# simonfuhrmann/mve

Measured on NVIDIA H100. Metric: mvs_depth_pixels_per_second, higher is better.
Workload: dtype f32

## Files before the change

mve_b200/csrc/b200mvs.cu:

```cuda
#include "../../include/b200mvs.h"
#include "patch_opt.cuh"
#include "patch_warp.cuh"
#include "patch_thread.cuh"

#include <algorithm>
#include <cmath>
#include <cstdarg>
#include <cstdio>
#include <cstring>
#include <cstdlib>
#include <map>
#include <chrono>
#include <ctime>
#include <mutex>
#include <string>
#include <thread>
#include <atomic>
#include <vector>

using namespace b200mvs;

namespace {

thread_local std::string g_create_error;
// ... 941 lines not shown
    {
        same_camera = v.valid && !v.lv.empty() && v.w == w && v.h == h && v.flen == flen && v.paspect == paspect && v.pp[0] == pp[0] && v.pp[1] == pp[1] &&
                      std::memcmp(v.rot, rot, sizeof(v.rot)) == 0 && std::memcmp(v.trans, trans, sizeof(v.trans)) == 0;
        if (!same_camera) { std::lock_guard<std::mutex> pl(ctx->plan_mtx); ctx->plans.clear(); }
    }
    if (!same_camera) {
        v.valid = false;
        v.has_image = false;
        v.w = w; v.h = h; v.flen = flen; v.paspect = paspect; v.pp[0] = pp[0]; v.pp[1] = pp[1];
        std::memcpy(v.rot, rot, sizeof(v.rot));
        std::memcpy(v.trans, trans, sizeof(v.trans));
        v.campos[0] = -rot[0] * trans[0] - rot[3] * trans[1] - rot[6] * trans[2];
        v.campos[1] = -rot[1] * trans[0] - rot[4] * trans[1] - rot[7] * trans[2];
        v.campos[2] = -rot[2] * trans[0] - rot[5] * trans[1] - rot[8] * trans[2];
        for (int r = 0; r < 3; ++r) {
            v.w2c[4 * r] = rot[3 * r]; v.w2c[4 * r + 1] = rot[3 * r + 1]; v.w2c[4 * r + 2] = rot[3 * r + 2]; v.w2c[4 * r + 3] = trans[r];
        }
        v.lv.clear();
        float ppx = pp[0], ppy = pp[1];
        int cw = w, chh = h;
        auto push_level = [&]() {
            HostLevel L; L.w = cw; L.h = chh; L.pitch = (cw + 3) & ~3;
            fill_calibration(v, ppx, ppy, (float)cw, (float)chh, L.proj, L.invproj);
            v.lv.push_back(L);
        };
        push_level();
        while (std::min(cw, chh) >= 30) {
            if (cw % 2 == 1) ppx = ppx * float(cw) / float(cw + 1);
            if (chh % 2 == 1) ppy = ppy * float(chh) / float(chh + 1);
            cw = (cw + 1) / 2; chh = (chh + 1) / 2;
            push_level();
        }
    }
    if ((int)v.lv.size() > MAX_LEVELS) return fail(ctx, B200MVS_ERR_UNSUPPORTED, "image too large: %d pyramid levels", (int)v.lv.size());
    if (!d_src) {
        if (v.d_base) { cudaFree(v.d_base); v.d_base = nullptr; v.bytes = 0; }
        v.has_image = false;
        v.valid = true;
        ctx->views_dirty = true;
        return 0;
    }
    size_t total = 0;
    for (HostLevel& L : v.lv) total += (size_t)L.pitch * L.h;
    const size_t need = total * (sizeof(uchar4) + sizeof(uint4));
    if (!v.d_base || v.bytes != need) {
        if (v.d_base) { cudaFree(v.d_base); v.d_base = nullptr; }
        CK(cudaMalloc(&v.d_base, need));
        v.bytes = need;
        ctx->views_dirty = true;
    }
    size_t off = 0;
    uint4* qbase = reinterpret_cast<uint4*>(v.d_base + total);
    for (HostLevel& L : v.lv) { L.d_img = v.d_base + off; L.d_quad = qbase + off; off += (size_t)L.pitch * L.h; }
    const dim3 blk(32, 8);
    k_import_rgb<<<dim3((w + 31) / 32, (h + 7) / 8), blk, 0, stream>>>(d_src, w, h, ch, v.lv[0].d_img, v.lv[0].pitch);
    const float w1 = std::exp(-0.5f / (2.0f * 1.0f)), w2 = std::exp(-2.5f / (2.0f * 1.0f)), w3 = std::exp(-4.5f / (2.0f * 1.0f));
    for (size_t i = 1; i < v.lv.size(); ++i) {
        const HostLevel& a = v.lv[i - 1];
        const HostLevel& b = v.lv[i];
        k_half_gaussian<<<dim3((b.w + 31) / 32, (b.h + 7) / 8), blk, 0, stream>>>(a.d_img, a.w, a.h, a.pitch, b.d_img, b.w, b.h, b.pitch, w1, w2, w3);
    }
    for (const HostLevel& L : v.lv)
        k_make_quads<<<dim3((L.w + 31) / 32, (L.h + 7) / 8), blk, 0, stream>>>(L.d_img, L.w, L.h, L.pitch, L.d_quad);
    CK(cudaGetLastError());
    v.valid = true;
    v.has_image = true;
    ctx->views_dirty = true;
    return 0;
}

int sync_view_params(b200mvs_ctx* ctx)
{
    if (!ctx->views_dirty) return 0;
    std::vector<ViewParams> hp(ctx->views.size());
    std::memset(hp.data(), 0, hp.size() * sizeof(ViewParams));
    for (size_t i = 0; i < ctx->views.size(); ++i) {
        const HostView& v = ctx->views[i];
        ViewParams& p = hp[i];
        p.valid = v.valid ? 1 : 0;
        if (!v.valid) continue;
        std::memcpy(p.campos, v.campos, 12);
        std::memcpy(p.w2c, v.w2c, 48);
        std::memcpy(p.rot, v.rot, 36);
        p.inv_ax0 = v.lv[0].invproj[0];
        p.nlevels = (int)v.lv.size();
        for (size_t l = 0; l < v.lv.size(); ++l) {
            const HostLevel& L = v.lv[l];
            p.lv[l].ax = L.proj[0]; p.lv[l].ay = L.proj[4]; p.lv[l].cx = L.proj[2]; p.lv[l].cy = L.proj[5];
            p.lv[l].w = L.w; p.lv[l].h = L.h; p.lv[l].pitch = L.pitch; p.lv[l].img = v.has_image ? L.d_img : nullptr;
            p.lv[l].quad = v.has_image ? L.d_quad : nullptr;
        }
    }
    CK(cudaMemcpyAsync(ctx->d_views, hp.data(), hp.size() * sizeof(ViewParams), cudaMemcpyHostToDevice, ctx->stream));
    CK(cudaStreamSynchronize(ctx->stream));
    ctx->views_dirty = false;
    return 0;
}

cudaEvent_t get_event(b200mvs_ctx* ctx, size_t i)
{
    while (ctx->ev_pool.size() <= i) { cudaEvent_t e; cudaEventCreate(&e); ctx->ev_pool.push_back(e); }
    return ctx->ev_pool[i];
}

int prepare_kernels(b200mvs_ctx* ctx)
{
    if (ctx->frontier_grid) return 0;
    CK(cudaFuncSetAttribute(k_frontier, cudaFuncAttributeMaxDynamicSharedMemorySize, (int)OPT_SMEM_BYTES));
    CK(cudaFuncSetAttribute(k_optimize, cudaFuncAttributeMaxDynamicSharedMemorySize, (int)OPT_SMEM_BYTES));
    int per_sm = 0, per_sm_opt = 0, sms = 0;
    CK(cudaOccupancyMaxActiveBlocksPerMultiprocessor(&per_sm, k_frontier, OPT_TPB, OPT_SMEM_BYTES));
    CK(cudaOccupancyMaxActiveBlocksPerMultiprocessor(&per_sm_opt, k_optimize, OPT_TPB, OPT_SMEM_BYTES));
    CK(cudaDeviceGetAttribute(&sms, cudaDevAttrMultiProcessorCount, ctx->device));
    if (per_sm < 1 || per_sm_opt < 1) return fail(ctx, B200MVS_ERR_CUDA, "patch-optimisation kernels do not fit on an SM");
    ctx->optimize_grid = per_sm_opt * sms;
    ctx->frontier_grid = per_sm * sms;
    return 0;
}

int make_job(b200mvs_ctx* ctx, const b200mvs_settings& s, int ref, const std::vector<int>& gsel, JobParams& J)
{
    const HostView& rv = ctx->views[ref];
    if (s.scale >= (int)rv.lv.size()) return fail(ctx, B200MVS_ERR_INVALID_ARG, "Invalid scale factor");
    const HostLevel& L = rv.lv[s.scale];
    std::memset(&J, 0, sizeof(J));
    J.ref_view = ref; J.W = L.w; J.H = L.h; J.n_global = (int)gsel.size();
    for (size_t k = 0; k < gsel.size(); ++k) J.gview[k] = gsel[k];
    J.ki0 = L.invproj[0]; J.ki2 = L.invproj[2]; J.ki4 = L.invproj[4]; J.ki5 = L.invproj[5];
    J.ref_img = L.d_img; J.ref_pitch = L.pitch;
    return 0;
}

unsigned ids_to_slots(const std::vector<int>& gsel, const int32_t* ids, int n, bool* ok)
{
    unsigned s = 0xFFFFFFFFu;
    std::vector<int> slots;
    for (int k = 0; k < n; ++k) {
        auto it = std::lower_bound(gsel.begin(), gsel.end(), (int)ids[k]);
        if (it == gsel.end() || *it != ids[k]) { *ok = false; return s; }
        slots.push_back((int)(it - gsel.begin()));
    }
    std::sort(slots.begin(), slots.end());
    for (size_t k = 0; k < slots.size() && k < 4; ++k) s = (s & ~(0xFFu << (8 * k))) | ((unsigned)slots[k] << (8 * k));
    *ok = true;
    return s;
}

}

extern "C" {

const char* b200mvs_version(void) { return "b200mvs 0.1 (sm_90a)"; }

void b200mvs_default_settings(b200mvs_settings* s)
{
    if (!s) return;
    s->filter_width = 5; s->min_ncc = 0.3f; s->min_parallax = 10.0f; s->accept_ncc = 0.6f; s->min_refine_diff = 0.001f;
    s->max_iterations = 20; s->nr_recon_neighbors = 4; s->global_vs_max = 20; s->scale = 0; s->use_color_scale = 1;
    for (int i = 0; i < 3; ++i) { s->aabb_min[i] = -3.402823466e+38f; s->aabb_max[i] = 3.402823466e+38f; }
    s->frontier_band = 0.f; s->frontier_topk = 0;
}

const char* b200mvs_last_error(const b200mvs_ctx* ctx) { return ctx ? ctx->err.c_str() : g_create_error.c_str(); }

int b200mvs_create(int device, int n_views, b200mvs_ctx** out)
{
    b200mvs_ctx* ctx = nullptr;
    if (!out || n_views <= 0) return fail(nullptr, B200MVS_ERR_INVALID_ARG, "b200mvs_create: bad arguments");
    *out = nullptr;
    if (device == B200MVS_DEVICE_NONE) {
        ctx = new b200mvs_ctx();
        ctx->device = B200MVS_DEVICE_NONE;
        ctx->views.resize(n_views);
        *out = ctx;
        return 0;
    }
    int ndev = 0;
    cudaError_t e = cudaGetDeviceCount(&ndev);
    if (e != cudaSuccess || ndev == 0)
        return fail(nullptr, B200MVS_ERR_CUDA, "no CUDA device available (%s); b200mvs has no CPU fallback", cudaGetErrorString(e));
    if (device < 0 || device >= ndev) return fail(nullptr, B200MVS_ERR_INVALID_ARG, "device %d out of range (%d devices)", device, ndev);
    e = cudaSetDevice(device);
    if (e != cudaSuccess) return fail(nullptr, B200MVS_ERR_CUDA, "cudaSetDevice: %s", cudaGetErrorString(e));
    ctx = new b200mvs_ctx();
    ctx->device = device;
    ctx->views.resize(n_views);
    auto bail = [&](const char* what, cudaError_t ce) {
        fail(nullptr, B200MVS_ERR_CUDA, "%s: %s", what, cudaGetErrorString(ce));
        delete ctx;
        return B200MVS_ERR_CUDA;
    };
    if ((e = cudaStreamCreateWithFlags(&ctx->stream, cudaStreamNonBlocking)) != cudaSuccess) return bail("cudaStreamCreate", e);
    if ((e = cudaMalloc(&ctx->d_views, sizeof(ViewParams) * n_views)) != cudaSuccess) return bail("cudaMalloc(views)", e);
    if ((e = cudaMalloc(&ctx->d_lut, 256 * sizeof(float))) != cudaSuccess) return bail("cudaMalloc(lut)", e);
    if ((e = cudaMallocHost(&ctx->h_counters, sizeof(unsigned long long) * 4096)) != cudaSuccess) return bail("cudaMallocHost", e);
    if ((e = cudaHostAlloc(&ctx->h_mirror, sizeof(unsigned long long) * 8192, cudaHostAllocMapped)) != cudaSuccess) return bail("cudaHostAlloc", e);
    float lut[256];
    for (int i = 0; i < 256; ++i) {
        const double x = i / 255.0;
        lut[i] = (float)((i <= 0.04045 * 255.0) ? x / 12.92 : std::pow((x + 0.055) / 1.055, 2.4));
    }
    if ((e = cudaMemcpy(ctx->d_lut, lut, sizeof(lut), cudaMemcpyHostToDevice)) != cudaSuccess) return bail("cudaMemcpy(lut)", e);
    *out = ctx;
    return 0;
}

void b200mvs_destroy(b200mvs_ctx* ctx)
{
    if (!ctx) return;
    if (ctx->device == B200MVS_DEVICE_NONE) { delete ctx; return; }
    cudaSetDevice(ctx->device);
    for (HostView& v : ctx->views) if (v.d_base) cudaFree(v.d_base);
    if (ctx->d_views) cudaFree(ctx->d_views);
    if (ctx->d_lut) cudaFree(ctx->d_lut);
    if (ctx->h_counters) cudaFreeHost(ctx->h_counters);
    if (ctx->h_mirror) cudaFreeHost(ctx->h_mirror);
    for (b200mvs_ctx::Stage& S : ctx->stage) {
        if (S.host) cudaFreeHost(S.host);
        if (S.dev) cudaFree(S.dev);
        if (S.done) cudaEventDestroy(S.done);
    }
    ctx->ent_a.release(); ctx->ent_b.release(); ctx->run_in.release(); ctx->run_sorted.release(); ctx->tile_cnt.release(); ctx->tile_off.release(); ctx->run_out.release(); ctx->written.release();
    ctx->counters.release(); ctx->d_jobs.release(); ctx->d_settings.release(); ctx->maps.release();
    ctx->ctl.release(); ctx->hist.release(); ctx->thr_bin.release(); ctx->job_cancel.release(); ctx->job_run.release();
    for (cudaEvent_t e : ctx->ev_pool) cudaEventDestroy(e);
    if (ctx->stream) cudaStreamDestroy(ctx->stream);
    delete ctx;
}

int b200mvs_upload_view(b200mvs_ctx* ctx, int id, const uint8_t* rgb, int w, int h, int channels,
                        float flen, float paspect, const float ppoint[2], const float rot[9], const float trans[3])
{
    if (!ctx) return B200MVS_ERR_INVALID_ARG;
    std::lock_guard<std::mutex> lk(ctx->mtx);
    if (ctx->device == B200MVS_DEVICE_NONE) return fail(ctx, B200MVS_ERR_CUDA, "planning context (B200MVS_DEVICE_NONE): no CUDA device, b200mvs has no CPU fallback");
    if (id < 0 || id >= (int)ctx->views.size() || !rgb || w < 2 || h < 2 || !ppoint || !rot || !trans)
        return fail(ctx, B200MVS_ERR_INVALID_ARG, "b200mvs_upload_view: bad arguments");
    if (channels < 1 || channels > 4) return fail(ctx, B200MVS_ERR_INVALID_ARG, "Image with invalid number of channels");
    CK(cudaSetDevice(ctx->device));
    const size_t bytes = (size_t)w * h * channels;
    b200mvs_ctx::Stage& S = ctx->stage[ctx->stage_next++ & 1u];
    if (S.busy) { CK(cudaEventSynchronize(S.done)); S.busy = false; }
    if (S.cap < bytes) {
        if (S.host) cudaFreeHost(S.host);
        if (S.dev) cudaFree(S.dev);
        S.host = nullptr; S.dev = nullptr; S.cap = 0;
        CK(cudaMallocHost(&S.host, bytes));
        CK(cudaMalloc(&S.dev, bytes));
        S.cap = bytes;
    }
    if (!S.done) CK(cudaEventCreateWithFlags(&S.done, cudaEventDisableTiming));
    std::memcpy(S.host, rgb, bytes);
    CK(cudaMemcpyAsync(S.dev, S.host, bytes, cudaMemcpyHostToDevice, ctx->stream));
    const int rc = upload_common(ctx, id, S.dev, w, h, channels, flen, paspect, ppoint, rot, trans, ctx->stream);
    CK(cudaEventRecord(S.done, ctx->stream));
    S.busy = true;
    return rc;
}

int b200mvs_upload_view_device(b200mvs_ctx* ctx, int id, const uint8_t* rgb_dev, int w, int h,
                               float flen, float paspect, const float ppoint[2], const float rot[9], const float trans[3],
                               void* cuda_stream)
{
    if (!ctx) return B200MVS_ERR_INVALID_ARG;
    std::lock_guard<std::mutex> lk(ctx->mtx);
    if (ctx->device == B200MVS_DEVICE_NONE) return fail(ctx, B200MVS_ERR_CUDA, "planning context (B200MVS_DEVICE_NONE): no CUDA device, b200mvs has no CPU fallback");
    if (id < 0 || id >= (int)ctx->views.size() || !rgb_dev || w < 2 || h < 2 || !ppoint || !rot || !trans)
        return fail(ctx, B200MVS_ERR_INVALID_ARG, "b200mvs_upload_view_device: bad arguments");
    CK(cudaSetDevice(ctx->device));
    cudaStream_t s = cuda_stream ? (cudaStream_t)cuda_stream : ctx->stream;
    int rc = upload_common(ctx, id, rgb_dev, w, h, 3, flen, paspect, ppoint, rot, trans, s);
    cudaError_t e = cudaStreamSynchronize(s);
    if (!rc && e != cudaSuccess) rc = fail(ctx, B200MVS_ERR_CUDA, "upload sync: %s", cudaGetErrorString(e));
    return rc;
}

int b200mvs_set_view_camera(b200mvs_ctx* ctx, int id, int w, int h, float flen, float paspect, const float ppoint[2],
                            const float rot[9], const float trans[3])
{
    if (!ctx) return B200MVS_ERR_INVALID_ARG;
    std::lock_guard<std::mutex> lk(ctx->mtx);
    if (id < 0 || id >= (int)ctx->views.size() || w < 2 || h < 2 || !ppoint || !rot || !trans)
        return fail(ctx, B200MVS_ERR_INVALID_ARG, "b200mvs_set_view_camera: bad arguments");
    if (ctx->device != B200MVS_DEVICE_NONE) CK(cudaSetDevice(ctx->device));
    return upload_common(ctx, id, nullptr, w, h, 3, flen, paspect, ppoint, rot, trans, ctx->stream);
}

int b200mvs_set_features(b200mvs_ctx* ctx, int n, const float* pos, const int32_t* off, const int32_t* ids)
{
    if (!ctx) return B200MVS_ERR_INVALID_ARG;
    std::lock_guard<std::mutex> lk(ctx->mtx);
    if (n < 0 || (n > 0 && (!pos || !off || !ids))) return fail(ctx, B200MVS_ERR_INVALID_ARG, "b200mvs_set_features: bad arguments");
    { std::lock_guard<std::mutex> pl(ctx->plan_mtx); ctx->plans.clear(); }
    ctx->feats.resize(n);
    for (int i = 0; i < n; ++i) {
        std::memcpy(ctx->feats[i].pos, pos + 3 * i, 12);
        ctx->feats[i].refs.assign(ids + off[i], ids + off[i + 1]);
    }
    ctx->view_feats.assign(ctx->views.size(), std::vector<int>());
    for (int i = 0; i < n; ++i)
        for (int vid : ctx->feats[i].refs)
            if (vid >= 0 && vid < (int)ctx->views.size()) {
                std::vector<int>& vf = ctx->view_feats[vid];
                if (vf.empty() || vf.back() != i) vf.push_back(i);
            }
    return 0;
// ... 452 lines not shown
```

mve_b200/csrc/patch_thread.cuh:

```cuda
#pragma once
#include "patch_opt.cuh"

namespace b200mvs {

struct PatchT {
    const DevSettings* st;
    const ViewParams* views;
#if defined(B200MVS_HOST_EMU)
    const float* lut_tab;
    unsigned lane4;
#endif
    const JobParams* job;
    unsigned xy;
    float u0x, u0y, u0z;
    float uax, uay, uaz;
    float ubx, uby, ubz;
    float c0x, c0y, c0z;
    float mx0, mx1, mx2;
    float crx, cry, crz;
    float cpx, cpy, cpz;
    float mfp, inv_mfp;
    float mm, inv_mm, sqrDevX;
    float depth, dzI, dzJ;
    unsigned avail;
    int iter;
    unsigned n_sets;
    unsigned pk;
    unsigned selp;
    float cs[MAX_LOCAL][3];
    float ncc[MAX_LOCAL];


    struct PassOut { float num, den, nX0, nX1, nX2; };
    enum Stage { LVS_CTOR, CTOR, FIRST, PRE, POST, LVS_REPL, REPL, DONE };
    enum : unsigned {
        F_REF_OK = 1u << 0,
        F_OPTI = 1u << 1, F_CONVERGED = 1u << 2, F_LVS_OK = 1u << 3, F_VIEW_REMOVED = 1u << 4, F_WAS_NORMAL = 1u << 5,
        F_NORMAL = 1u << 6, F_SINGULAR = 1u << 7, F_HAS_NORMAL = 1u << 8, F_HAS_NCC = 1u << 9
    };
    static constexpr int SH_STAGE = 10, SH_NSEL = 13, SH_COL = 16, SH_DER = 20, SH_DF = 24;
    __device__ __forceinline__ bool is(unsigned f) const { return (pk & f) != 0u; }
    __device__ __forceinline__ void put(unsigned f, bool v) { pk = v ? (pk | f) : (pk & ~f); }
    __device__ __forceinline__ int stage() const { return (int)((pk >> SH_STAGE) & 7u); }
    __device__ __forceinline__ void set_stage(int v) { pk = (pk & ~(7u << SH_STAGE)) | ((unsigned)v << SH_STAGE); }
    __device__ __forceinline__ int nsel() const { return (int)((pk >> SH_NSEL) & 7u); }
    __device__ __forceinline__ void set_nsel(int v) { pk = (pk & ~(7u << SH_NSEL)) | ((unsigned)v << SH_NSEL); }
    __device__ __forceinline__ int sel(int k) const { return (int)((selp >> (8 * k)) & 0xFFu); }
    __device__ __forceinline__ int px() const { return (int)(xy & 0xFFFFu); }
    __device__ __forceinline__ int py() const { return (int)(xy >> 16); }

    template <typename T> static __device__ __forceinline__ T get4(const T (&a)[MAX_LOCAL], int k)
    {
        return k == 0 ? a[0] : (k == 1 ? a[1] : (k == 2 ? a[2] : a[3]));
    }
    template <typename T> static __device__ __forceinline__ void set4(T (&a)[MAX_LOCAL], int k, T v)
    {
#pragma unroll
        for (int i = 0; i < MAX_LOCAL; ++i) if (i == k) a[i] = v;
    }

    __device__ __forceinline__ unsigned lane_offset() const
    {
#if defined(B200MVS_HOST_EMU)
        return lane4;
#else
        return (threadIdx.x & 31u) << 2;
#endif
    }
    __device__ __forceinline__ const float* table() const
    {
#if defined(B200MVS_HOST_EMU)
        return lut_tab;
#else
        extern __shared__ float b200mvs_dyn_smem[];
        return b200mvs_dyn_smem;
#endif
    }

    __device__ __forceinline__ void sample_ray(float di, float dj, float& ux, float& uy, float& uz, float& inv) const
    {
        ux = u0x + di * uax + dj * ubx;
        uy = u0y + di * uay + dj * uby;
        uz = u0z + di * uaz + dj * ubz;
        inv = rsqrt_fast(ux * ux + uy * uy + uz * uz);
    }

    __device__ __forceinline__ void compute_points()
    {
        bool bad = false;
#pragma unroll 5
        for (int k = 0; k < NS; ++k) {
            const float t = depth + (float)(k % 5 - 2) * dzI + (float)(k / 5 - 2) * dzJ;
            bad |= t <= 0.f;
        }
        if (bad) pk &= ~F_REF_OK;
        cpx = c0x + depth * crx;
        cpy = c0y + depth * cry;
        cpz = c0z + depth * crz;
        const ViewParams* rv = &views[job->ref_view];
        const float z = __ldg(&rv->w2c[8]) * cpx + __ldg(&rv->w2c[9]) * cpy + __ldg(&rv->w2c[10]) * cpz + __ldg(&rv->w2c[11]);
        mfp = z * job->ki0;
        inv_mfp = rcp_fast(mfp);
    }

    __device__ __forceinline__ void init_sampler(int x, int y)
    {
        const float* const lut_tab = table();
        const unsigned lane4 = lane_offset();
        pk &= ~F_REF_OK; mm = 0.f; inv_mm = 0.f; sqrDevX = 0.f;
        mx0 = mx1 = mx2 = 0.f;
        crx = cry = crz = cpx = cpy = cpz = mfp = inv_mfp = 0.f;
        if (x - 2 < 0 || y - 2 < 0 || x + 2 > job->W - 1 || y + 2 > job->H - 1) return;
        {
            const ViewParams* rv = &views[job->ref_view];
            const float r0 = __ldg(&rv->rot[0]), r1 = __ldg(&rv->rot[1]), r2 = __ldg(&rv->rot[2]), r3 = __ldg(&rv->rot[3]), r4 = __ldg(&rv->rot[4]);
            const float r5 = __ldg(&rv->rot[5]), r6 = __ldg(&rv->rot[6]), r7 = __ldg(&rv->rot[7]), r8 = __ldg(&rv->rot[8]);
            const float vx = job->ki0 * ((float)x + 0.5f) + job->ki2, vy = job->ki4 * ((float)y + 0.5f) + job->ki5;
            u0x = r0 * vx + r3 * vy + r6; u0y = r1 * vx + r4 * vy + r7; u0z = r2 * vx + r5 * vy + r8;
            uax = r0 * job->ki0; uay = r1 * job->ki0; uaz = r2 * job->ki0;
            ubx = r3 * job->ki4; uby = r4 * job->ki4; ubz = r5 * job->ki4;
            c0x = __ldg(&rv->campos[0]); c0y = __ldg(&rv->campos[1]); c0z = __ldg(&rv->campos[2]);
            const float inv = rsqrt_fast(u0x * u0x + u0y * u0y + u0z * u0z);
            crx = u0x * inv; cry = u0y * inv; crz = u0z * inv;
        }
        pk |= F_REF_OK;
        const uchar4* row = job->ref_img + (size_t)(y - 2) * job->ref_pitch + (x - 2);
        float s0 = 0.f, s1 = 0.f, s2 = 0.f;
#pragma unroll 1
        for (int j = 0; j < 5; ++j) {
#pragma unroll
            for (int i = 0; i < 5; ++i) {
                const unsigned t = reinterpret_cast<const unsigned*>(row)[i];
                s0 += lut_k<0>(lut_tab, lane4, t); s1 += lut_k<1>(lut_tab, lane4, t); s2 += lut_k<2>(lut_tab, lane4, t);
            }
            row += job->ref_pitch;
        }
        mm = (s0 + s1 + s2) / (3.f * NS);
        if (mm < 0.01f || mm > 0.99f) { pk &= ~F_REF_OK; return; }
        inv_mm = 1.f / mm;
        mx0 = (s0 * inv_mm) / (float)NS; mx1 = (s1 * inv_mm) / (float)NS; mx2 = (s2 * inv_mm) / (float)NS;
        row = job->ref_img + (size_t)(y - 2) * job->ref_pitch + (x - 2);
        float dev = 0.f;
#pragma unroll 1
        for (int j = 0; j < 5; ++j) {
#pragma unroll
            for (int i = 0; i < 5; ++i) {
                const unsigned t = reinterpret_cast<const unsigned*>(row)[i];
                const float e0 = lut_k<0>(lut_tab, lane4, t) * inv_mm - mx0, e1 = lut_k<1>(lut_tab, lane4, t) * inv_mm - mx1, e2 = lut_k<2>(lut_tab, lane4, t) * inv_mm - mx2;
                dev += e0 * e0 + e1 * e1 + e2 * e2;
            }
            row += job->ref_pitch;
        }
        sqrDevX = dev;
        compute_points();
    }

    __device__ __forceinline__ void update()
    {
        pk |= F_REF_OK;
        compute_points();
    }

    __device__ __forceinline__ void pass(bool candidates, bool cs_pending, bool want_ncc, bool want_normal, float* cand, PassOut& po)
    {
        const float* const lut_tab = table();
        const unsigned lane4 = lane_offset();
        const float u0x = this->u0x, u0y = this->u0y, u0z = this->u0z, uax = this->uax, uay = this->uay, uaz = this->uaz;
        const float ubx = this->ubx, uby = this->uby, ubz = this->ubz;
        const float depth = this->depth, dzI = this->dzI, dzJ = this->dzJ;
        const float mx0 = this->mx0, mx1 = this->mx1, mx2 = this->mx2, mm = this->mm, inv_mm = this->inv_mm;
        const JobParams* const job = this->job;
        float num = 0.f, den = 0.f;
        double D0 = 0.0, D1 = 0.0, D2 = 0.0, D3 = 0.0, D4 = 0.0, D5 = 0.0, E0 = 0.0, E1 = 0.0, E2 = 0.0;
        bool cs_active = cs_pending && st->use_color_scale;
        if (!candidates) pk &= want_ncc ? ~((0xFFu << SH_COL) | (0xFu << SH_DF)) : ~(0xFFu << SH_COL);
        const int count = candidates ? job->n_global : nsel();
        const int x0 = px(), y0 = py();
        const float pv0 = mx0 * mm, pv1 = mx1 * mm, pv2 = mx2 * mm;
#pragma unroll 1
        for (int k = 0; k < count; ++k) {
            int slot = k;
            if (candidates) { if (!((avail >> k) & 1u)) continue; }
            else slot = sel(k);
            const ViewParams* V = &views[job->gview[slot]];
            ++n_sets;
            float c0 = 1.f, c1 = 1.f, c2 = 1.f;
            if (!candidates) {
                c0 = k == 0 ? cs[0][0] : (k == 1 ? cs[1][0] : (k == 2 ? cs[2][0] : cs[3][0]));
                c1 = k == 0 ? cs[0][1] : (k == 1 ? cs[1][1] : (k == 2 ? cs[2][1] : cs[3][1]));
                c2 = k == 0 ? cs[0][2] : (k == 1 ? cs[1][2] : (k == 2 ? cs[2][2] : cs[3][2]));
            }
            unsigned r = 0u;
            float A0x = 0.f, A0y = 0.f, A0z = 0.f, W0x = 0.f, W0y = 0.f, W0z = 0.f, Wax = 0.f, Way = 0.f, Waz = 0.f, Wbx = 0.f, Wby = 0.f, Wbz = 0.f;
            float Lax = 0.f, Lay = 0.f, Lcx = 0.f, Lcy = 0.f, wm1 = 0.f, hm1 = 0.f, dd = 0.f, step = 0.f;
            int Lpitch = 0;
            const uint4* Lquad = nullptr;
            bool dok = false;
            {
                const float4 wa = __ldg(reinterpret_cast<const float4*>(&V->w2c[0]));
                const float4 wb = __ldg(reinterpret_cast<const float4*>(&V->w2c[4]));
                const float4 wc = __ldg(reinterpret_cast<const float4*>(&V->w2c[8]));
                A0x = wa.x * c0x + wa.y * c0y + wa.z * c0z + wa.w;
                A0y = wb.x * c0x + wb.y * c0y + wb.z * c0z + wb.w;
                A0z = wc.x * c0x + wc.y * c0y + wc.z * c0z + wc.w;
                W0x = wa.x * u0x + wa.y * u0y + wa.z * u0z; W0y = wb.x * u0x + wb.y * u0y + wb.z * u0z; W0z = wc.x * u0x + wc.y * u0y + wc.z * u0z;
                Wax = wa.x * uax + wa.y * uay + wa.z * uaz; Way = wb.x * uax + wb.y * uay + wb.z * uaz; Waz = wc.x * uax + wc.y * uay + wc.z * uaz;
                Wbx = wa.x * ubx + wa.y * uby + wa.z * ubz; Wby = wb.x * ubx + wb.y * uby + wb.z * ubz; Wbz = wc.x * ubx + wc.y * uby + wc.z * ubz;
                const float nz = wc.x * cpx + wc.y * cpy + wc.z * cpz + wc.w;
                const float nfp = nz * __ldg(&V->inv_ax0);
                if (mfp > 0.f && !(nfp <= 0.f)) {
                    float ratio = nfp * inv_mfp;
                    int l = 0;
                    while (ratio < 0.5f) { ++l; ratio *= 2.f; }
                    const int nl = __ldg(&V->nlevels);
                    if (l > nl - 1) l = nl - 1;
                    const float4 kk = __ldg(reinterpret_cast<const float4*>(&V->lv[l].ax));
                    const int4 g = __ldg(reinterpret_cast<const int4*>(&V->lv[l].w));
                    Lax = kk.x; Lay = kk.y; Lcx = kk.z; Lcy = kk.w; wm1 = (float)(g.x - 1); hm1 = (float)(g.y - 1); Lpitch = g.z;
                    Lquad = reinterpret_cast<const uint4*>(__ldg(reinterpret_cast<const unsigned long long*>(&V->lv[l].quad)));
                    const float inv0 = rsqrt_fast(u0x * u0x + u0y * u0y + u0z * u0z);
                    const float sa = depth * inv0, sb = (depth + 1.f) * inv0;
                    const float hz1 = A0z + sa * W0z, hz2 = A0z + sb * W0z;
                    const float i1 = rcp_fast(hz1), i2 = rcp_fast(hz2);
                    const float ddx = (Lax * (A0x + sb * W0x) + Lcx * hz2) * i2 - (Lax * (A0x + sa * W0x) + Lcx * hz1) * i1;
                    const float ddy = (Lay * (A0y + sb * W0y) + Lcy * hz2) * i2 - (Lay * (A0y + sa * W0y) + Lcy * hz1) * i1;
                    const float dd2 = ddx * ddx + ddy * ddy;
                    dd = dd2 * rsqrt_fast(dd2);
                    dok = dd > 0.f;
                    step = rcp_fast(dd);
                    r = dok ? 3u : 1u;
                }
            }
            const bool need_ncc = candidates || want_ncc;
            const bool cs_view = !candidates && cs_active;
            float nccv = -1.f;
#pragma unroll 1
            for (int rep = 0; rep < 2 && r != 0u; ++rep) {
                const bool second = rep == 1;
                if (second && !(cs_view && want_normal && (r & 2u))) break;
                const bool do_ncc = !second && need_ncc;
                const bool do_cs = !second && cs_view;
                const bool gn_direct = !candidates && (r & 2u) && (second || !cs_view);
                const bool gn_sums = !candidates && (r & 2u) && !second && cs_view && !want_normal;
                float S1a = 0.f, S1b = 0.f, S1c = 0.f, S2a = 0.f, S2b = 0.f, S2c = 0.f, Sen = 0.f;
                float X0 = 0.f, X1 = 0.f, X2 = 0.f, X3 = 0.f, X4 = 0.f, X5 = 0.f, X6 = 0.f, X7 = 0.f, X8 = 0.f, X9 = 0.f, X10 = 0.f,
                      X11 = 0.f, X12 = 0.f, X13 = 0.f, X14 = 0.f;
                float &Mna = X0, &Mnb = X1, &Mnc = X2, &Nna = X3, &Nnb = X4, &Nnc = X5;
                float &Dma = X6, &Dmb = X7, &Dmc = X8, &Dna = X9, &Dnb = X10, &Dnc = X11, &Dda = X12, &Ddb = X13, &Ddc = X14;
                float &vnum = X0, &vden = X1;
                float &A0 = X2, &A1 = X3, &A2 = X4, &A3 = X5, &A4 = X6, &A5 = X7, &B0 = X8, &B1 = X9, &B2 = X10;
                bool oob = false;
                const uchar4* mptr = job->ref_img + (size_t)(y0 - 2) * job->ref_pitch + (x0 - 2);
                const int mskip = job->ref_pitch - 5;
                float ndi = -2.f, ndj = -2.f;
                float nfx = 0.f, nfy = 0.f, ngx = 0.f, ngy = 0.f;
                uint4 nQ = make_uint4(0u, 0u, 0u, 0u);
                unsigned nmt = 0u;
                bool nvalid = false;
#define B200MVS_STAGE_NEXT() do { \
                    const float ux_ = u0x + ndi * uax + ndj * ubx, uy_ = u0y + ndi * uay + ndj * uby, uz_ = u0z + ndi * uaz + ndj * ubz; \
                    const float inv_ = rsqrt_fast(ux_ * ux_ + uy_ * uy_ + uz_ * uz_); \
                    const float t_ = depth + ndi * dzI + ndj * dzJ; \
                    const float s1_ = t_ * inv_; \
                    const float wx_ = W0x + ndi * Wax + ndj * Wbx, wy_ = W0y + ndi * Way + ndj * Wby, wz_ = W0z + ndi * Waz + ndj * Wbz; \
                    const float hx_ = A0x + s1_ * wx_, hy_ = A0y + s1_ * wy_, hz_ = A0z + s1_ * wz_; \
                    const float ih_ = rcp_fast(hz_); \
                    const float qx_ = (Lax * hx_ + Lcx * hz_) * ih_ - 0.5f; \
                    const float qy_ = (Lay * hy_ + Lcy * hz_) * ih_ - 0.5f; \
                    nvalid = qx_ > 0.f && qx_ < wm1 && qy_ > 0.f && qy_ < hm1; \
                    if (nvalid) { \
                        ngx = 0.f; ngy = 0.f; \
                        if (dok) { \
                            const float s2_ = s1_ + step * inv_; \
                            const float kx_ = A0x + s2_ * wx_, ky_ = A0y + s2_ * wy_, kz_ = A0z + s2_ * wz_; \
                            const float ik_ = rcp_fast(kz_); \
                            ngx = (Lax * kx_ + Lcx * kz_) * ik_ - 0.5f - qx_; \
                            ngy = (Lay * ky_ + Lcy * kz_) * ik_ - 0.5f - qy_; \
                        } \
                        const int left_ = (int)floorf(qx_), top_ = (int)floorf(qy_); \
                        nfx = qx_ - (float)left_; nfy = qy_ - (float)top_; \
                        noff = (unsigned)top_ * (unsigned)Lpitch + (unsigned)left_; \
                        nQ = __ldg(Lquad + noff); \
                        nmt = *reinterpret_cast<const unsigned*>(mptr); \
                    } \
                } while (0)
                unsigned noff = 0u;
                B200MVS_STAGE_NEXT();
#ifdef B200MVS_T1_UNROLL2
#pragma unroll 2
#else
#pragma unroll 1
#endif
                for (int k = 0; k < NS; ++k) {
                    if (!nvalid) { oob = true; break; }
                    const float di = ndi, dj = ndj, fx = nfx, fy = nfy, gx = ngx, gy = ngy;
                    const uint4 Q = nQ;
                    const unsigned mt = nmt;
                    if (k + 1 < NS) {
                        ndi += 1.f; ++mptr;
                        if (ndi > 2.f) { ndi = -2.f; ndj += 1.f; mptr += mskip; }
                        B200MVS_STAGE_NEXT();
                    }
                    {
                        const float m[3] = {lut_k<0>(lut_tab, lane4, mt) * inv_mm, lut_k<1>(lut_tab, lane4, mt) * inv_mm, lut_k<2>(lut_tab, lane4, mt) * inv_mm};
                        float a[3], b[3], c[3], e[3];
                        a[0] = lut_k<0>(lut_tab, lane4, Q.x); a[1] = lut_k<1>(lut_tab, lane4, Q.x); a[2] = lut_k<2>(lut_tab, lane4, Q.x);
                        b[0] = lut_k<0>(lut_tab, lane4, Q.y); b[1] = lut_k<1>(lut_tab, lane4, Q.y); b[2] = lut_k<2>(lut_tab, lane4, Q.y);
                        c[0] = lut_k<0>(lut_tab, lane4, Q.z); c[1] = lut_k<1>(lut_tab, lane4, Q.z); c[2] = lut_k<2>(lut_tab, lane4, Q.z);
                        e[0] = lut_k<0>(lut_tab, lane4, Q.w); e[1] = lut_k<1>(lut_tab, lane4, Q.w); e[2] = lut_k<2>(lut_tab, lane4, Q.w);
                        float n[3], d[3];
#pragma unroll
                        for (int ch = 0; ch < 3; ++ch) {
                            const float x0_ = (1.f - fx) * a[ch] + fx * b[ch];
                            const float x3_ = (1.f - fx) * c[ch] + fx * e[ch];
                            n[ch] = (1.f - fy) * x0_ + fy * x3_;
                            const float der = gx * (b[ch] - a[ch]) + gy * (c[ch] - a[ch]) + (gy * fx + gx * fy) * (a[ch] - b[ch] - c[ch] + e[ch]);
                            d[ch] = dok ? der * dd : 0.f;
                        }
                        if (do_ncc) {
                            const float y0_ = n[0] - pv0, y1_ = n[1] - pv1, y2_ = n[2] - pv2;
                            S1a += y0_; S1b += y1_; S1c += y2_;
                            S2a += y0_ * y0_; S2b += y1_ * y1_; S2c += y2_ * y2_;
                            Sen += (m[0] - mx0) * y0_ + (m[1] - mx1) * y1_ + (m[2] - mx2) * y2_;
                        }
                        if (do_cs) {
                            Mna += m[0] * n[0]; Mnb += m[1] * n[1]; Mnc += m[2] * n[2];
                            Nna += n[0] * n[0]; Nnb += n[1] * n[1]; Nnc += n[2] * n[2];
                        }
                        if (gn_sums) {
                            Dma += d[0] * m[0]; Dmb += d[1] * m[1]; Dmc += d[2] * m[2];
                            Dna += d[0] * n[0]; Dnb += d[1] * n[1]; Dnc += d[2] * n[2];
                            Dda += d[0] * d[0]; Ddb += d[1] * d[1]; Ddc += d[2] * d[2];
                        }
                        if (gn_direct) {
                            const float g0 = c0 * d[0], g1 = c1 * d[1], g2 = c2 * d[2];
                            const float r0 = m[0] - c0 * n[0], r1 = m[1] - c1 * n[1], r2 = m[2] - c2 * n[2];
                            vnum += g0 * r0 + g1 * r1 + g2 * r2;
                            vden += g0 * g0 + g1 * g1 + g2 * g2;
                            if (want_normal) {
                                const float gg[3] = {g0, g1, g2};
                                const float rr[3] = {r0, r1, r2};
#pragma unroll
                                for (int ch = 0; ch < 3; ++ch) {
                                    const float a0 = gg[ch];
                                    const float a1 = di * a0;
                                    const float a2 = dj * a0;
                                    A0 += a0 * a0; A1 += a0 * a1; A2 += a0 * a2;
                                    A3 += a1 * a1; A4 += a1 * a2; A5 += a2 * a2;
                                    B0 += a0 * rr[ch]; B1 += a1 * rr[ch]; B2 += a2 * rr[ch];
                                }
                            }
                        }
                    }
                }
#undef B200MVS_STAGE_NEXT
                if (oob) { r = 0u; break; }
                if (do_ncc) {
                    const float inv_n = 1.f / (float)NS;
                    const float sqrDevY = (S2a - S1a * S1a * inv_n) + (S2b - S1b * S1b * inv_n) + (S2c - S1c * S1c * inv_n);
                    const float p = sqrDevX * sqrDevY;
                    nccv = p > 0.f ? Sen * rsqrt_fast(p) : -1.f;
                }
                if (do_cs) {
                    float cc[3] = {c0, c1, c2};
                    const float ab[3] = {Mna - c0 * Nna, Mnb - c1 * Nnb, Mnc - c2 * Nnc};
                    const float aa[3] = {Nna, Nnb, Nnc};
#pragma unroll
                    for (int ch = 0; ch < 3; ++ch) {
                        if ((double)fabsf(aa[ch]) > 1e-6) {
                            cc[ch] += ab[ch] * rcp_fast(aa[ch]);
                            if ((double)cc[ch] > 1e3) pk &= ~F_OPTI;
                        } else
                            pk &= ~F_OPTI;
                    }
                    c0 = cc[0]; c1 = cc[1]; c2 = cc[2];
#pragma unroll
                    for (int i = 0; i < MAX_LOCAL; ++i) if (i == k) { cs[i][0] = c0; cs[i][1] = c1; cs[i][2] = c2; }
                }
                if (gn_sums) {
                    const float vn = c0 * (Dma - c0 * Dna) + c1 * (Dmb - c1 * Dnb) + c2 * (Dmc - c2 * Dnc);
                    const float vd = c0 * c0 * Dda + c1 * c1 * Ddb + c2 * c2 * Ddc;
                    vnum = vn; vden = vd;
                }
                if (gn_direct || gn_sums) {
                    num += vnum; den += vden;
                    if (want_normal && gn_direct) {
                        D0 += (double)A0; D1 += (double)A1; D2 += (double)A2; D3 += (double)A3; D4 += (double)A4; D5 += (double)A5;
                        E0 += (double)B0; E1 += (double)B1; E2 += (double)B2;
                    }
                }
            }
            if (!candidates) {
                if (r & 1u) pk |= 1u << (SH_COL + k);
                if (r & 2u) pk |= 1u << (SH_DER + k);
                if (cs_active && !(r & 1u)) cs_active = false;
                if (want_ncc) {
                    const float v = (r & 1u) ? nccv : -1.f;
                    if (fabsf(v - get4(ncc, k)) > st->min_refine_diff) pk |= 1u << (SH_DF + k);
                    set4(ncc, k, v);
                }
            } else {
                const float v = (r & 1u) ? nccv : -1.f;
                if (v < st->min_ncc) avail &= ~(1u << k);
                else cand[k] = v;
            }
        }
        if (candidates) return;
        po.num = num; po.den = den;
        put(F_HAS_NORMAL, want_normal);
        put(F_HAS_NCC, want_ncc);
        if (want_normal) {
            const double m[9] = {D0, D1, D2, D1, D3, D4, D2, D4, D5};
            const double det = m[0] * m[4] * m[8] + m[1] * m[5] * m[6] + m[2] * m[3] * m[7]
                             - m[2] * m[4] * m[6] - m[1] * m[3] * m[8] - m[0] * m[5] * m[7];
            put(F_SINGULAR, det == 0.0);
            double inv[9];
            inv[0] = m[4] * m[8] - m[5] * m[7];
            inv[1] = m[2] * m[7] - m[1] * m[8];
            inv[2] = m[1] * m[5] - m[2] * m[4];
            inv[3] = m[5] * m[6] - m[3] * m[8];
            inv[4] = m[0] * m[8] - m[2] * m[6];
            inv[5] = m[2] * m[3] - m[0] * m[5];
            inv[6] = m[3] * m[7] - m[4] * m[6];
            inv[7] = m[1] * m[6] - m[0] * m[7];
            inv[8] = m[0] * m[4] - m[1] * m[3];
#pragma unroll
            for (int q = 0; q < 9; ++q) inv[q] /= det;
            po.nX0 = (float)(inv[0] * E0 + inv[1] * E1 + inv[2] * E2);
            po.nX1 = (float)(inv[3] * E0 + inv[4] * E1 + inv[5] * E2);
            po.nX2 = (float)(inv[6] * E0 + inv[7] * E1 + inv[8] * E2);
        }
    }

    __device__ __forceinline__ bool all_der_ok() const { return ((pk >> SH_DER) & 0xFu) == ((1u << nsel()) - 1u); }

    __device__ __forceinline__ bool depth_step(const PassOut& po)
    {
        if (!all_der_ok()) { pk &= ~F_OPTI; return false; }
        if (po.den > 0.f) {
            depth += po.num / po.den;
            update();
            put(F_OPTI, is(F_REF_OK));
            return true;
        }
        return false;
    }

    __device__ __forceinline__ bool normal_step(const PassOut& po)
    {
        if (!all_der_ok()) { pk &= ~F_OPTI; return false; }
        if (is(F_SINGULAR)) { pk &= ~F_OPTI; return false; }
        dzI += po.nX1; dzJ += po.nX2; depth += po.nX0;
        update();
        put(F_OPTI, is(F_REF_OK));
        return true;
    }

    __device__ __forceinline__ void sel_erase_mask(unsigned mask)
    {
        const int n = nsel();
        int cnt = 0;
        unsigned packed = 0xFFFFFFFFu;
#pragma unroll
        for (int k = 0; k < MAX_LOCAL; ++k) {
            if (k < n && !((mask >> k) & 1u)) {
                const unsigned s8 = (selp >> (8 * k)) & 0xFFu;
                const float a = cs[k][0], b = cs[k][1], c = cs[k][2], v = ncc[k];
                packed = (packed & ~(0xFFu << (8 * cnt))) | (s8 << (8 * cnt));
#pragma unroll
                for (int q = 0; q < MAX_LOCAL; ++q) if (q == cnt) { cs[q][0] = a; cs[q][1] = b; cs[q][2] = c; ncc[q] = v; }
                ++cnt;
            }
        }
        selp = packed;
        set_nsel(cnt);
    }
    __device__ __forceinline__ void sel_insert(int slot, float cs_init)
    {
        const int n = nsel();
        int pos = 0;
#pragma unroll
        for (int k = 0; k < MAX_LOCAL; ++k) if (k < n && sel(k) < slot) ++pos;
#pragma unroll
        for (int q = MAX_LOCAL - 1; q > 0; --q)
            if (q > pos && q <= n) { cs[q][0] = cs[q - 1][0]; cs[q][1] = cs[q - 1][1]; cs[q][2] = cs[q - 1][2]; ncc[q] = ncc[q - 1]; }
#pragma unroll
        for (int q = 0; q < MAX_LOCAL; ++q) if (q == pos) { cs[q][0] = cs[q][1] = cs[q][2] = cs_init; ncc[q] = 0.f; }
        const unsigned low = pos == 0 ? 0u : (selp & (0xFFFFFFFFu >> (32 - 8 * pos)));
        const unsigned high = pos >= 3 ? 0u : ((selp >> (8 * pos)) << (8 * (pos + 1)));
        selp = low | ((unsigned)slot << (8 * pos)) | high;
        set_nsel(n + 1);
    }

    __device__ __forceinline__ void cand_geometry(int slot, float rdx, float rdy, float rdz,
                                                  float& vdx, float& vdy, float& vdz, float& epx, float& epy, float& epz, float& nfp) const
    {
        const ViewParams* V = &views[job->gview[slot]];
        vdx = cpx - __ldg(&V->campos[0]); vdy = cpy - __ldg(&V->campos[1]); vdz = cpz - __ldg(&V->campos[2]);
        const float nn = sqrtf(vdx * vdx + vdy * vdy + vdz * vdz);
        vdx /= nn; vdy /= nn; vdz /= nn;
        epx = vdy * rdz - vdz * rdy; epy = vdz * rdx - vdx * rdz; epz = vdx * rdy - vdy * rdx;
        const float en = sqrtf(epx * epx + epy * epy + epz * epz);
        epx /= en; epy /= en; epz /= en;
        const float z = __ldg(&V->w2c[8]) * cpx + __ldg(&V->w2c[9]) * cpy + __ldg(&V->w2c[10]) * cpz + __ldg(&V->w2c[11]);
        nfp = z * __ldg(&V->inv_ax0);
    }

    __device__ __forceinline__ void lvs_greedy(const float* cand)
    {
        const unsigned N = st->nr_recon_neighbors;
        const float cs_init = 1.f / mm;
        float rdx = cpx - c0x, rdy = cpy - c0y, rdz = cpz - c0z;
        {
            const float nn = sqrtf(rdx * rdx + rdy * rdy + rdz * rdz);
            rdx /= nn; rdy /= nn; rdz /= nn;
        }
        const int G = job->n_global;
        bool found = true;
        while ((unsigned)nsel() < N && found) {
            found = false;
            float maxScore = 0.f;
            int maxView = 0;
#pragma unroll 1
            for (int c = 0; c < G; ++c) {
                if (!((avail >> c) & 1u)) continue;
                float vdx, vdy, vdz, epx, epy, epz, nfp;
                cand_geometry(c, rdx, rdy, rdz, vdx, vdy, vdz, epx, epy, epz, nfp);
                float score = cand[c];
                if (mfp / nfp < 0.5f) score *= 0.01f;
                float dp = clamp1(rdx * vdx + rdy * vdy + rdz * vdz);
                score *= plx_weight(deg_acos(dp));
                const int ns = nsel();
#pragma unroll 1
                for (int k = 0; k < ns; ++k) {
                    float sx, sy, sz, ex, ey, ez, sfp;
                    cand_geometry(sel(k), rdx, rdy, rdz, sx, sy, sz, ex, ey, ez, sfp);
                    dp = clamp1(sx * vdx + sy * vdy + sz * vdz);
                    score *= plx_weight(deg_acos(dp));
                    dp = clamp1(epx * ex + epy * ey + epz * ez);
                    float angle = fabsf(deg_acos(dp));
                    if (angle > 90.f) angle = 180.f - angle;
// ... 156 lines not shown
```

Measured before the change: 54.61 million.

## Accumulate unified per-channel moment sums and derive NCC, color-scale and Gauss-Newton terms

Replaces the mode-specific accumulator sets (NCC, color scale, GN sums, GN direct) with one fixed set of per-channel moment sums computed every sample, from which NCC, color-scale and Gauss-Newton numerators and denominators are derived after the loop. The normal-equation accumulation is collapsed from per-channel terms to a per-pixel squared-gradient and residual scalar, and the derivative is always multiplied by dd (set to zero when invalid). The aim is to remove warp divergence between threads in different sweep modes and to cut per-sample arithmetic. The cost is extra accumulation work for modes that did not need all sums, more registers, and changed float rounding, since the sums are re-centered algebraically. An optional compile-time counter for sweep-mode mix is also added.

Result: faster. 56.44 million (median of 6 runs) (+3.4%).

```diff
diff --git a/mve_b200/csrc/b200mvs.cu b/mve_b200/csrc/b200mvs.cu
--- a/mve_b200/csrc/b200mvs.cu
+++ b/mve_b200/csrc/b200mvs.cu
@@ -1117,6 +1117,17 @@
 
 const char* b200mvs_version(void) { return "b200mvs 0.1 (sm_90a)"; }
 
+#if defined(B200MVS_SWEEP_MIX)
+int b200mvs_sweep_mix(uint64_t* out, int n)
+{
+    if (!out || n <= 0) return -1;
+    unsigned long long h[128];
+    if (cudaMemcpyFromSymbol(h, b200mvs::g_sweep_mix, sizeof(h)) != cudaSuccess) return -1;
+    for (int i = 0; i < n && i < 128; ++i) out[i] = h[i];
+    return 0;
+}
+#endif
+
 void b200mvs_default_settings(b200mvs_settings* s)
 {
     if (!s) return;
diff --git a/mve_b200/csrc/patch_thread.cuh b/mve_b200/csrc/patch_thread.cuh
--- a/mve_b200/csrc/patch_thread.cuh
+++ b/mve_b200/csrc/patch_thread.cuh
@@ -2,6 +2,23 @@
 #include "patch_opt.cuh"
 
 namespace b200mvs {
+
+#if defined(B200MVS_SWEEP_MIX) && !defined(B200MVS_HOST_EMU)
+__device__ unsigned long long g_sweep_mix[128];
+__device__ __forceinline__ void count_sweep_mix(unsigned kind)
+{
+    const unsigned act = __activemask();
+    const unsigned same = __match_any_sync(act, kind);
+    const int lane = (int)(threadIdx.x & 31u);
+    const unsigned firsts = __ballot_sync(act, (__ffs(same) - 1) == lane);
+    atomicAdd(&g_sweep_mix[64 + (kind & 63u)], 1ull);
+    if (lane == __ffs(act) - 1) {
+        atomicAdd(&g_sweep_mix[__popc(firsts) & 31], 1ull);
+        atomicAdd(&g_sweep_mix[32], 1ull);
+        atomicAdd(&g_sweep_mix[33], (unsigned long long)__popc(act));
+    }
+}
+#endif
 
 struct PatchT {
     const DevSettings* st;
@@ -168,7 +185,7 @@
         const float u0x = this->u0x, u0y = this->u0y, u0z = this->u0z, uax = this->uax, uay = this->uay, uaz = this->uaz;
         const float ubx = this->ubx, uby = this->uby, ubz = this->ubz;
         const float depth = this->depth, dzI = this->dzI, dzJ = this->dzJ;
-        const float mx0 = this->mx0, mx1 = this->mx1, mx2 = this->mx2, mm = this->mm, inv_mm = this->inv_mm;
+        const float inv_mm = this->inv_mm;
         const JobParams* const job = this->job;
         float num = 0.f, den = 0.f;
         double D0 = 0.0, D1 = 0.0, D2 = 0.0, D3 = 0.0, D4 = 0.0, D5 = 0.0, E0 = 0.0, E1 = 0.0, E2 = 0.0;
@@ -229,6 +246,7 @@
                     dok = dd > 0.f;
                     step = rcp_fast(dd);
                     r = dok ? 3u : 1u;
+                    if (!dok) dd = 0.f;
                 }
             }
             const bool need_ncc = candidates || want_ncc;
@@ -238,17 +256,19 @@
             for (int rep = 0; rep < 2 && r != 0u; ++rep) {
                 const bool second = rep == 1;
                 if (second && !(cs_view && want_normal && (r & 2u))) break;
-                const bool do_ncc = !second && need_ncc;
-                const bool do_cs = !second && cs_view;
-                const bool gn_direct = !candidates && (r & 2u) && (second || !cs_view);
-                const bool gn_sums = !candidates && (r & 2u) && !second && cs_view && !want_normal;
-                float S1a = 0.f, S1b = 0.f, S1c = 0.f, S2a = 0.f, S2b = 0.f, S2c = 0.f, Sen = 0.f;
-                float X0 = 0.f, X1 = 0.f, X2 = 0.f, X3 = 0.f, X4 = 0.f, X5 = 0.f, X6 = 0.f, X7 = 0.f, X8 = 0.f, X9 = 0.f, X10 = 0.f,
-                      X11 = 0.f, X12 = 0.f, X13 = 0.f, X14 = 0.f;
-                float &Mna = X0, &Mnb = X1, &Mnc = X2, &Nna = X3, &Nnb = X4, &Nnc = X5;
-                float &Dma = X6, &Dmb = X7, &Dmc = X8, &Dna = X9, &Dnb = X10, &Dnc = X11, &Dda = X12, &Ddb = X13, &Ddc = X14;
-                float &vnum = X0, &vden = X1;
-                float &A0 = X2, &A1 = X3, &A2 = X4, &A3 = X5, &A4 = X6, &A5 = X7, &B0 = X8, &B1 = X9, &B2 = X10;
+                const bool gn = !candidates && (r & 2u) && (second || !(cs_view && want_normal));
+                const bool nrm = gn && want_normal;
+#if defined(B200MVS_SWEEP_MIX) && !defined(B200MVS_HOST_EMU)
+                {
+                    const bool g_ = !candidates && (r & 2u);
+                    count_sweep_mix((!second && need_ncc ? 1u : 0u) | (!second && cs_view ? 2u : 0u) |
+                                    (g_ && !second && cs_view && !want_normal ? 4u : 0u) | (g_ && (second || !cs_view) ? 8u : 0u) |
+                                    (g_ && (second || !cs_view) && want_normal ? 16u : 0u) | (candidates ? 32u : 0u));
+                }
+#endif
+                float Sya = 0.f, Syb = 0.f, Syc = 0.f, Syya = 0.f, Syyb = 0.f, Syyc = 0.f, Smya = 0.f, Smyb = 0.f, Smyc = 0.f;
+                float Sdma = 0.f, Sdmb = 0.f, Sdmc = 0.f, Sdna = 0.f, Sdnb = 0.f, Sdnc = 0.f, Sdda = 0.f, Sddb = 0.f, Sddc = 0.f;
+                float A1 = 0.f, A2 = 0.f, A3 = 0.f, A4 = 0.f, A5 = 0.f, B1 = 0.f, B2 = 0.f;
                 bool oob = false;
                 const uchar4* mptr = job->ref_img + (size_t)(y0 - 2) * job->ref_pitch + (x0 - 2);
                 const int mskip = job->ref_pitch - 5;
@@ -315,53 +335,38 @@
                             const float x3_ = (1.f - fx) * c[ch] + fx * e[ch];
                             n[ch] = (1.f - fy) * x0_ + fy * x3_;
                             const float der = gx * (b[ch] - a[ch]) + gy * (c[ch] - a[ch]) + (gy * fx + gx * fy) * (a[ch] - b[ch] - c[ch] + e[ch]);
-                            d[ch] = dok ? der * dd : 0.f;
+                            d[ch] = der * dd;
                         }
-                        if (do_ncc) {
-                            const float y0_ = n[0] - pv0, y1_ = n[1] - pv1, y2_ = n[2] - pv2;
-                            S1a += y0_; S1b += y1_; S1c += y2_;
-                            S2a += y0_ * y0_; S2b += y1_ * y1_; S2c += y2_ * y2_;
-                            Sen += (m[0] - mx0) * y0_ + (m[1] - mx1) * y1_ + (m[2] - mx2) * y2_;
-                        }
-                        if (do_cs) {
-                            Mna += m[0] * n[0]; Mnb += m[1] * n[1]; Mnc += m[2] * n[2];
-                            Nna += n[0] * n[0]; Nnb += n[1] * n[1]; Nnc += n[2] * n[2];
-                        }
-                        if (gn_sums) {
-                            Dma += d[0] * m[0]; Dmb += d[1] * m[1]; Dmc += d[2] * m[2];
-                            Dna += d[0] * n[0]; Dnb += d[1] * n[1]; Dnc += d[2] * n[2];
-                            Dda += d[0] * d[0]; Ddb += d[1] * d[1]; Ddc += d[2] * d[2];
-                        }
-                        if (gn_direct) {
+                        const float y0_ = n[0] - pv0, y1_ = n[1] - pv1, y2_ = n[2] - pv2;
+                        Sya += y0_; Syb += y1_; Syc += y2_;
+                        Syya += y0_ * y0_; Syyb += y1_ * y1_; Syyc += y2_ * y2_;
+                        Smya += m[0] * y0_; Smyb += m[1] * y1_; Smyc += m[2] * y2_;
+                        Sdma += d[0] * m[0]; Sdmb += d[1] * m[1]; Sdmc += d[2] * m[2];
+                        Sdna += d[0] * n[0]; Sdnb += d[1] * n[1]; Sdnc += d[2] * n[2];
+                        Sdda += d[0] * d[0]; Sddb += d[1] * d[1]; Sddc += d[2] * d[2];
+                        if (nrm) {
                             const float g0 = c0 * d[0], g1 = c1 * d[1], g2 = c2 * d[2];
-                            const float r0 = m[0] - c0 * n[0], r1 = m[1] - c1 * n[1], r2 = m[2] - c2 * n[2];
-                            vnum += g0 * r0 + g1 * r1 + g2 * r2;
-                            vden += g0 * g0 + g1 * g1 + g2 * g2;
-                            if (want_normal) {
-                                const float gg[3] = {g0, g1, g2};
-                                const float rr[3] = {r0, r1, r2};
-#pragma unroll
-                                for (int ch = 0; ch < 3; ++ch) {
-                                    const float a0 = gg[ch];
-                                    const float a1 = di * a0;
-                                    const float a2 = dj * a0;
-                                    A0 += a0 * a0; A1 += a0 * a1; A2 += a0 * a2;
-                                    A3 += a1 * a1; A4 += a1 * a2; A5 += a2 * a2;
-                                    B0 += a0 * rr[ch]; B1 += a1 * rr[ch]; B2 += a2 * rr[ch];
-                                }
-                            }
+                            const float q = g0 * g0 + g1 * g1 + g2 * g2;
+                            const float s = g0 * (m[0] - c0 * n[0]) + g1 * (m[1] - c1 * n[1]) + g2 * (m[2] - c2 * n[2]);
+                            const float qi = di * q, qj = dj * q;
+                            A1 += qi; A2 += qj; A3 += di * qi; A4 += dj * qi; A5 += dj * qj;
+                            B1 += di * s; B2 += dj * s;
                         }
                     }
                 }
 #undef B200MVS_STAGE_NEXT
                 if (oob) { r = 0u; break; }
-                if (do_ncc) {
+                if (!second && need_ncc) {
                     const float inv_n = 1.f / (float)NS;
-                    const float sqrDevY = (S2a - S1a * S1a * inv_n) + (S2b - S1b * S1b * inv_n) + (S2c - S1c * S1c * inv_n);
+                    const float sqrDevY = (Syya - Sya * Sya * inv_n) + (Syyb - Syb * Syb * inv_n) + (Syyc - Syc * Syc * inv_n);
+                    const float Sen = (Smya - mx0 * Sya) + (Smyb - mx1 * Syb) + (Smyc - mx2 * Syc);
                     const float p = sqrDevX * sqrDevY;
                     nccv = p > 0.f ? Sen * rsqrt_fast(p) : -1.f;
                 }
-                if (do_cs) {
+                if (!second && cs_view) {
+                    const float Mna = Smya + pv0 * ((float)NS * mx0), Mnb = Smyb + pv1 * ((float)NS * mx1), Mnc = Smyc + pv2 * ((float)NS * mx2);
+                    const float Nna = Syya + pv0 * (2.f * Sya + (float)NS * pv0), Nnb = Syyb + pv1 * (2.f * Syb + (float)NS * pv1);
+                    const float Nnc = Syyc + pv2 * (2.f * Syc + (float)NS * pv2);
                     float cc[3] = {c0, c1, c2};
                     const float ab[3] = {Mna - c0 * Nna, Mnb - c1 * Nnb, Mnc - c2 * Nnc};
                     const float aa[3] = {Nna, Nnb, Nnc};
@@ -377,16 +382,13 @@
 #pragma unroll
                     for (int i = 0; i < MAX_LOCAL; ++i) if (i == k) { cs[i][0] = c0; cs[i][1] = c1; cs[i][2] = c2; }
                 }
-                if (gn_sums) {
-                    const float vn = c0 * (Dma - c0 * Dna) + c1 * (Dmb - c1 * Dnb) + c2 * (Dmc - c2 * Dnc);
-                    const float vd = c0 * c0 * Dda + c1 * c1 * Ddb + c2 * c2 * Ddc;
-                    vnum = vn; vden = vd;
-                }
-                if (gn_direct || gn_sums) {
-                    num += vnum; den += vden;
-                    if (want_normal && gn_direct) {
-                        D0 += (double)A0; D1 += (double)A1; D2 += (double)A2; D3 += (double)A3; D4 += (double)A4; D5 += (double)A5;
-                        E0 += (double)B0; E1 += (double)B1; E2 += (double)B2;
+                if (gn) {
+                    const float vn = c0 * (Sdma - c0 * Sdna) + c1 * (Sdmb - c1 * Sdnb) + c2 * (Sdmc - c2 * Sdnc);
+                    const float vd = c0 * c0 * Sdda + c1 * c1 * Sddb + c2 * c2 * Sddc;
+                    num += vn; den += vd;
+                    if (nrm) {
+                        D0 += (double)vd; D1 += (double)A1; D2 += (double)A2; D3 += (double)A3; D4 += (double)A4; D5 += (double)A5;
+                        E0 += (double)vn; E1 += (double)B1; E2 += (double)B2;
                     }
                 }
             }
```
